# anonymousauthors001/SGS-GNN

Measured on AMD Instinct MI355X. Metric: sampled edges/sec + training steps/sec, Reddit hybrid 20% sparsity, higher is better.
Workload: dtype f32

## Files before the change

include/sgs_hip.h:

```cpp
#ifndef SGS_HIP_H_
#define SGS_HIP_H_

#include <stddef.h>
#include <stdint.h>

#ifdef __cplusplus
extern "C" {
#endif

#define SGS_ABI_VERSION 1

#define SGS_OK 0
#define SGS_EINVAL (-1)
#define SGS_EWORKSPACE (-2)
#define SGS_EHIP (-3)

typedef void* sgs_stream_t;

int sgs_abi_version(void);
const char* sgs_last_error(void);

int sgs_rng_set_epoch_buffer(const uint64_t* epoch_dev);
int sgs_exp_noise(uint64_t seed, uint64_t stream_id, int64_t E, float* noise, sgs_stream_t stream);
int sgs_dropout_keep(uint64_t seed, uint32_t site, int64_t rows, int64_t cols, float p, uint8_t* keep,
// ... 104 lines not shown
                          const int32_t* loop_eid, const int64_t* edge_index, const float* Hn, float* dw,
                          sgs_stream_t stream);

#define SGS_ACT_NONE 0
#define SGS_ACT_RELU 1
#define SGS_ACT_RELU_DROPOUT 2
int sgs_spmm_csr(const float* X, int64_t N, int64_t D, int64_t nnz, const int32_t* ptr, const int32_t* col, const float* val,
                 const float* diag, const float* bias, int act, float p_drop, uint64_t seed, uint32_t site, float* Y,
                 sgs_stream_t stream);

int sgs_sddmm_csr(const float* A, const float* B, int64_t N, int64_t D, int64_t nnz, const int32_t* ptr, const int32_t* col,
                  const int32_t* eid, float* g, float* gdiag, sgs_stream_t stream);

int sgs_spmm_csr_variant(int64_t N, int64_t D, int64_t nnz, int aligned16);
int sgs_sddmm_csr_variant(int64_t N, int64_t D, int64_t nnz, int aligned16);

int sgs_act_bwd(const float* dY, const float* Y, int64_t n, int act, float p_drop, float* dZ, sgs_stream_t stream);
size_t sgs_colsum_workspace_bytes(int64_t N, int64_t D);
int sgs_colsum(const float* A, int64_t N, int64_t D, float* out, void* ws, size_t ws_bytes, sgs_stream_t stream);
int sgs_act_bwd_colsum(const float* dY, const float* Y, int64_t N, int64_t D, int act, float p_drop, float* dZ, float* colsum, void* ws,
                       size_t ws_bytes, sgs_stream_t stream);

int sgs_colsum_variant(int64_t N, int64_t D, int fused_act);

int sgs_gcn_pair_ok(int64_t N, int64_t nnz, int64_t D);
int sgs_spmm_csr_next(const float* X, int64_t N, int64_t D, int64_t nnz, const int32_t* ptr, const int32_t* col, const float* val,
                      const float* diag, const float* bias, int act, float p_drop, uint64_t seed, uint32_t site, const float* Wn, int64_t Dn,
                      float* Y, float* Z, sgs_stream_t stream);
int sgs_spmm_csr_bwd_prev(const float* dZ, int64_t N, int64_t D, int64_t nnz, const int32_t* ptr, const int32_t* col, const float* val,
                          const float* diag, const float* W, int64_t Dp, const float* Yp, int act, float p_drop, float* dX, float* dZp,
// ... 370 lines not shown
```

sgs-gnn_amd/csrc/gcn.hip:

```cpp
#include "sgs_common.h"

namespace sgs {
size_t graph_sort_workspace_bytes(int64_t n, int64_t N);
size_t graph_src_sorted_workspace_bytes(int64_t n, int64_t N);
int graph_build_src_sorted(const int64_t* ei, int64_t n, int64_t N, int32_t* in_ptr, int32_t* in_src, int32_t* in_eid, int32_t* out_ptr,
                           int32_t* out_dst, int32_t* out_eid, int32_t* loop_eid, int32_t* unsorted_flag, void* ws, size_t ws_bytes,
                           hipStream_t stream);
int graph_build_by_sort(const int64_t* ei, int64_t n, int64_t N, int32_t* in_ptr, int32_t* in_src, int32_t* in_eid, int32_t* out_ptr,
                        int32_t* out_dst, int32_t* out_eid, int32_t* loop_eid, void* ws, size_t ws_bytes, hipStream_t stream);
}

namespace sgs {
namespace {

constexpr int kT = 256;
constexpr int kMaxLdsRow = 8192;

__global__ void __launch_bounds__(kT) count_degrees(const int64_t* __restrict__ ei, int64_t n_edges, int* __restrict__ cnt_in,
                                                   int* __restrict__ cnt_out, int* __restrict__ loop_eid) {
    const int64_t e = static_cast<int64_t>(blockIdx.x) * kT + threadIdx.x;
    if (e >= n_edges) return;
    const int s = static_cast<int>(ei[e]), d = static_cast<int>(ei[n_edges + e]);
    atomicAdd(&cnt_in[d], 1);
    atomicAdd(&cnt_out[s], 1);
// ... 591 lines not shown
                        ? y * drop_scale : 0.f;
            o[v] = y;
        }
        *reinterpret_cast<V*>(Y + i * D + c0) = *reinterpret_cast<V*>(o);
    }
}
template <int VEC, int LPR>
__global__ void __launch_bounds__(kT) spmm_csr(const float* __restrict__ X, int64_t N, int64_t D, const int* __restrict__ ptr,
                                              const int* __restrict__ col, const float* __restrict__ val,
                                              const float* __restrict__ diag, const float* __restrict__ bias, int act,
                                              float drop_scale, uint32_t drop_thresh, uint64_t seed, uint32_t site,
                                              const uint64_t* __restrict__ epoch, float* __restrict__ Y) {
    spmm_csr_body<VEC, LPR>(X, N, D, ptr, col, val, diag, bias, act, drop_scale, drop_thresh, seed, site, epoch, Y);
}

template <int VEC, int NW>
__device__ __forceinline__ void spmm_csr_rowblock_body(const float* __restrict__ X, int64_t N, int64_t D, const int* __restrict__ ptr,
                                                       const int* __restrict__ col, const float* __restrict__ val,
                                                       const float* __restrict__ diag, const float* __restrict__ bias, int act,
                                                       float drop_scale, uint32_t drop_thresh, uint64_t seed, uint32_t site,
                                                       const uint64_t* __restrict__ epoch, float* __restrict__ Y) {
    using V = typename VecT<VEC>::type;
    __shared__ float part[NW][64 * VEC];
    seed = fold_epoch(seed, epoch);
    const int lane = threadIdx.x & 63, wave = threadIdx.x >> 6;
    const int64_t i = blockIdx.x;
    const int b = ptr[i], e = ptr[i + 1];
    const float dg = diag ? diag[i] : 0.f;
    const uint32_t rkey = dropout_row_key(seed, site, static_cast<uint64_t>(i));
    for (int64_t cbase = 0; cbase < D; cbase += 64 * VEC) {
        const int64_t c0 = cbase + static_cast<int64_t>(lane) * VEC;
        const bool in = c0 < D;
        float acc[VEC];
#pragma unroll
        for (int v = 0; v < VEC; ++v) acc[v] = 0.f;
        if (in) {
            int k = b + wave;
            for (; k + 7 * NW < e; k += 8 * NW) {
                int j[8]; float w[8]; V x[8];
#pragma unroll
                for (int u = 0; u < 8; ++u) { j[u] = col[k + NW * u]; w[u] = val[k + NW * u]; }
#pragma unroll
                for (int u = 0; u < 8; ++u) x[u] = *reinterpret_cast<const V*>(X + static_cast<int64_t>(j[u]) * D + c0);
#pragma unroll
                for (int u = 0; u < 8; ++u) {
                    float xv[VEC];
                    *reinterpret_cast<V*>(xv) = x[u];
#pragma unroll
                    for (int v = 0; v < VEC; ++v) acc[v] = fmaf(w[u], xv[v], acc[v]);
                }
            }
// ... 11 lines not shown
        const int t = threadIdx.x;
        if (t < 64 * VEC && cbase + t < D) {
            const int64_t c = cbase + t;
            float y = 0.f;
#pragma unroll
            for (int g = 0; g < NW; g += 4) y += (part[g][t] + part[g + 1][t]) + (part[g + 2][t] + part[g + 3][t]);
            if (diag) y = fmaf(dg, X[i * D + c], y);
            if (bias) y += bias[c];
            if (act != SGS_ACT_NONE) y = fmaxf(y, 0.f);
            if (act == SGS_ACT_RELU_DROPOUT) y = dropout_keep_col(rkey, static_cast<uint32_t>(c), drop_thresh) ? y * drop_scale : 0.f;
            Y[i * D + c] = y;
        }
        __syncthreads();
    }
}
template <int VEC, int NW>
__global__ void __launch_bounds__(64 * NW) spmm_csr_rowblock(const float* __restrict__ X, int64_t N, int64_t D, const int* __restrict__ ptr,
                                                       const int* __restrict__ col, const float* __restrict__ val,
                                                       const float* __restrict__ diag, const float* __restrict__ bias, int act,
                                                       float drop_scale, uint32_t drop_thresh, uint64_t seed, uint32_t site,
                                                       const uint64_t* __restrict__ epoch, float* __restrict__ Y) {
    spmm_csr_rowblock_body<VEC, NW>(X, N, D, ptr, col, val, diag, bias, act, drop_scale, drop_thresh, seed, site, epoch, Y);
}

template <int VEC, int LPR>
__global__ void __launch_bounds__(kT) sddmm_csr(const float* __restrict__ A, const float* __restrict__ B, int64_t N, int64_t D,
                                               const int* __restrict__ ptr, const int* __restrict__ col,
                                               const int* __restrict__ eid, float* __restrict__ g, float* __restrict__ gdiag) {
    using V = typename VecT<VEC>::type;
    constexpr int RPB = kT / LPR;
    const int sub = threadIdx.x % LPR;
    const int64_t i = static_cast<int64_t>(blockIdx.x) * RPB + threadIdx.x / LPR;
    const bool live = i < N;
    const int b = live ? ptr[i] : 0, e = live ? ptr[i + 1] : 0;
    int trips = e - b + 1;
    for (int o = 32; o > 0; o >>= 1) trips = max(trips, __shfl_xor(trips, o, 64));
    for (int t = 0; t < trips; ++t) {
// ... 260 lines not shown
__global__ void __launch_bounds__(kT) multi_norm_weights(const float* __restrict__ w, int64_t q, int64_t N, const int* __restrict__ in_ptr,
                                                        const int* __restrict__ in_src, const int* __restrict__ in_eid, const float* __restrict__ dis,
                                                        const float* __restrict__ loopw, float* __restrict__ what_in, float* __restrict__ what_loop) {
    const int64_t d = blockIdx.y;
    norm_weights_body(N, w ? w + d * q : nullptr, N, q, in_ptr + d * (N + 1), in_src + d * q, in_eid + d * q, nullptr, nullptr, nullptr, dis + d * N,
                      loopw + d * N, what_in + d * q, nullptr, what_loop + d * N);
}
template <int VEC, int LPR>
__global__ void __launch_bounds__(kT) multi_spmm_csr(const float* __restrict__ X, int64_t xs, int64_t N, int64_t D, int64_t nnz,
                                                    const int* __restrict__ ptr, const int* __restrict__ col, const float* __restrict__ val,
                                                    const float* __restrict__ diag, const float* __restrict__ bias, int act, float* __restrict__ Y) {
    const int64_t d = blockIdx.y;
    spmm_csr_body<VEC, LPR>(X + d * xs, N, D, ptr + d * (N + 1), col + d * nnz, val + d * nnz, diag ? diag + d * N : nullptr, bias, act, 1.0f, 0u,
                            uint64_t(0), 0u, nullptr, Y + d * N * D);
}
template <int VEC, int NW>
__global__ void __launch_bounds__(64 * NW) multi_spmm_csr_rowblock(const float* __restrict__ X, int64_t xs, int64_t N, int64_t D, int64_t nnz,
                                                                 const int* __restrict__ ptr, const int* __restrict__ col,
                                                                 const float* __restrict__ val, const float* __restrict__ diag,
                                                                 const float* __restrict__ bias, int act, float* __restrict__ Y) {
    const int64_t d = blockIdx.y;
    spmm_csr_rowblock_body<VEC, NW>(X + d * xs, N, D, ptr + d * (N + 1), col + d * nnz, val + d * nnz, diag ? diag + d * N : nullptr, bias, act,
                                    1.0f, 0u, uint64_t(0), 0u, nullptr, Y + d * N * D);
}

enum { kPairCol = 0, kPairFwd = 1, kPairBwd = 2 };
constexpr int kPairMaxD = 512;
constexpr int kPairWlds = 12288;
constexpr int kPairWpre = kPairWlds / 1024;
template <class FY, class FW>
__device__ __forceinline__ float lib_gemm_dot(int K, FY y, FW w) {
    const int Kmain = K / 16 * 16;
    float z = 0.f;
    if (Kmain > 0) {
        float ya[8], wa[8];
#pragma unroll
        for (int u = 0; u < 8; ++u) { const int k = 2 * (u & 3) + (u >> 2); ya[u] = y(k); wa[u] = w(k); }
        for (int b = 0; b < Kmain; b += 8) {
            const int nb = b + 8 < Kmain ? b + 8 : b;
            float yn[8], wn[8];
#pragma unroll
            for (int u = 0; u < 8; ++u) { const int k = nb + 2 * (u & 3) + (u >> 2); yn[u] = y(k); wn[u] = w(k); }
#pragma unroll
            for (int u = 0; u < 8; ++u) z = fmaf(ya[u], wa[u], z);
#pragma unroll
            for (int u = 0; u < 8; ++u) { ya[u] = yn[u]; wa[u] = wn[u]; }
        }
    }
    for (int k = Kmain; k < K; ++k) z = fmaf(y(k), w(k), z);
    return z;
}
template <int VEC, int NW, int MODE, int GU = 8>
__device__ __forceinline__ void spmm_rowgroup_pair_body(const float* __restrict__ X, int64_t N, int64_t D, const int* __restrict__ ptr,
                                                        const int* __restrict__ col, const float* __restrict__ val,
                                                        const float* __restrict__ diag, const float* __restrict__ bias, int act,
                                                        float drop_scale, uint32_t drop_thresh, uint64_t seed, uint32_t site,
                                                        const uint64_t* __restrict__ epoch, float* __restrict__ Y,
                                                        const float* __restrict__ Wn, int64_t Dn, const float* __restrict__ Yp,
                                                        float* __restrict__ Zn, int ncs, float* __restrict__ colsum) {
    using V = typename VecT<VEC>::type;
    constexpr int RG = 16 / NW;
    __shared__ float part[RG][NW][64 * VEC];
    __shared__ __align__(16) float ys[RG * kPairMaxD];
    __shared__ float wl[MODE == kPairFwd ? kPairWlds : 1];
    if (MODE != kPairFwd && static_cast<int>(blockIdx.x) < ncs) {
        if (D % 4 == 0) colsum_small_v4_body<false>(X, nullptr, N, D, SGS_ACT_NONE, 1.f, nullptr, colsum, blockIdx.x);
        else            colsum_small_body<false>(X, nullptr, N, D, SGS_ACT_NONE, 1.f, nullptr, colsum, blockIdx.x);
// ... 17 lines not shown
    const bool wlds = MODE == kPairFwd && Dn * D <= kPairWlds;
    float wpre[MODE == kPairFwd ? kPairWpre : 1];
    if (MODE == kPairFwd && wlds) {
#pragma unroll
        for (int u = 0; u < kPairWpre; ++u) {
            const int64_t idx = threadIdx.x + 1024 * u;
            wpre[u] = idx < Dn * D ? Wn[idx] : 0.f;
        }
    }
    for (int64_t cbase = 0; cbase < D; cbase += 64 * VEC) {
        const int64_t c0 = cbase + static_cast<int64_t>(lane) * VEC;
        const bool in = c0 < D;
        float acc[VEC];
#pragma unroll
        for (int v = 0; v < VEC; ++v) acc[v] = 0.f;
        if (in) {
            int k = b + wave;
            for (; k + (GU - 1) * NW < e; k += GU * NW) {
                int j[GU]; float w[GU]; V x[GU];
#pragma unroll
                for (int u = 0; u < GU; ++u) { j[u] = col[k + NW * u]; w[u] = val[k + NW * u]; }
#pragma unroll
                for (int u = 0; u < GU; ++u) x[u] = *reinterpret_cast<const V*>(X + static_cast<int64_t>(j[u]) * D + c0);
#pragma unroll
                for (int u = 0; u < GU; ++u) {
                    float xv[VEC];
                    *reinterpret_cast<V*>(xv) = x[u];
#pragma unroll
                    for (int v = 0; v < VEC; ++v) acc[v] = fmaf(w[u], xv[v], acc[v]);
                }
            }
// ... 44 lines not shown
            Zn[ir * Dn + o] = wlds ? lib_gemm_dot(static_cast<int>(D), yk, [&](int k) { return wl[k * Dn + o]; })
                                   : lib_gemm_dot(static_cast<int>(D), yk, [&](int k) { return Wn[o * D + k]; });
        }
    } else if (MODE == kPairBwd) {
        for (int64_t idx = threadIdx.x; idx < RG * Dn; idx += 1024) {
            const int r = static_cast<int>(idx / Dn);
            const int64_t ep = idx - r * Dn, ir = row0 + r;
            if (ir >= N) break;
            const float* yr = ys + r * D;
            float a = lib_gemm_dot(static_cast<int>(D), [&](int c) { return yr[c]; }, [&](int c) { return Wn[c * Dn + ep]; });
            if (act != SGS_ACT_NONE) a = (Yp[ir * Dn + ep] > 0.f) ? (act == SGS_ACT_RELU_DROPOUT ? a * drop_scale : a) : 0.f;
            Zn[ir * Dn + ep] = a;
        }
    }
}
template <int VEC, int NW, int MODE>
__global__ void __launch_bounds__(1024) spmm_rowgroup_pair(const float* __restrict__ X, int64_t N, int64_t D, const int* __restrict__ ptr,
                                                           const int* __restrict__ col, const float* __restrict__ val,
                                                           const float* __restrict__ diag, const float* __restrict__ bias, int act,
                                                           float drop_scale, uint32_t drop_thresh, uint64_t seed, uint32_t site,
                                                           const uint64_t* __restrict__ epoch, float* __restrict__ Y,
                                                           const float* __restrict__ Wn, int64_t Dn, const float* __restrict__ Yp,
                                                           float* __restrict__ Zn, int ncs, float* __restrict__ colsum) {
    spmm_rowgroup_pair_body<VEC, NW, MODE>(X, N, D, ptr, col, val, diag, bias, act, drop_scale, drop_thresh, seed, site, epoch, Y, Wn, Dn, Yp, Zn,
                                           ncs, colsum);
}

struct SpmmDualJob {
    const float* X;
    const int* ptr;
    const int* col;
    const float* val;
    const float* diag;
    float* Y;
    float* Z;
    int64_t nnz;
    uint64_t seed;
};
struct SpmmDualArgs {
    SpmmDualJob job[2];
};
template <int VEC, int NW>
__global__ void __launch_bounds__(64 * NW) spmm_csr_rowblock_dual(SpmmDualArgs a, int64_t N, int64_t D, const float* __restrict__ bias, int act,
                                                                  float drop_scale, uint32_t drop_thresh, uint32_t site,
                                                                  const uint64_t* __restrict__ epoch) {
    const SpmmDualJob& j = a.job[blockIdx.y];
    spmm_csr_rowblock_body<VEC, NW>(j.X, N, D, j.ptr, j.col, j.val, j.diag, bias, act, drop_scale, drop_thresh, j.seed, site, epoch, j.Y);
}
#ifndef SGS_DUAL_PAIR_CAPPED
#define SGS_DUAL_PAIR_CAPPED 1
#endif
constexpr int kDualPairWaves = SGS_DUAL_PAIR_CAPPED ? 8 : 4;
constexpr int dual_pair_gu(int vec) { return SGS_DUAL_PAIR_CAPPED && vec == 4 ? 4 : 8; }
template <int VEC, int NW>
__global__ void __launch_bounds__(1024, kDualPairWaves) spmm_rowgroup_pair_dual(SpmmDualArgs a, int64_t N, int64_t D,
                                                                                const float* __restrict__ bias, int act, float drop_scale,
                                                                                uint32_t drop_thresh, uint32_t site,
                                                                                const uint64_t* __restrict__ epoch,
                                                                                const float* __restrict__ Wn, int64_t Dn) {
    const SpmmDualJob& j = a.job[blockIdx.y];
    spmm_rowgroup_pair_body<VEC, NW, kPairFwd, dual_pair_gu(VEC)>(j.X, N, D, j.ptr, j.col, j.val, j.diag, bias, act, drop_scale, drop_thresh, j.seed,
                                                            site, epoch, j.Y, Wn, Dn, nullptr, j.Z, 0, nullptr);
}

inline int pick_lpr(int64_t D, int vec) {
    const int64_t need = (D + vec - 1) / vec;
    int lpr = 1;
    while (lpr < need && lpr < 64) lpr <<= 1;
    return lpr;
}

}
}

using namespace sgs;

#define DISPATCH_VEC_LPR(KERNEL, vec, lpr, grid_rows, ...)                                                       \
// ... 12 lines not shown
            }                                                                                                     \
        } else {                                                                                                  \
            switch (lpr) {                                                                                        \
                case 1: hipLaunchKernelGGL((KERNEL<1, 1>), _g, _b, 0, stream, __VA_ARGS__); break;                \
                case 2: hipLaunchKernelGGL((KERNEL<1, 2>), _g, _b, 0, stream, __VA_ARGS__); break;                \
                case 4: hipLaunchKernelGGL((KERNEL<1, 4>), _g, _b, 0, stream, __VA_ARGS__); break;                \
                case 8: hipLaunchKernelGGL((KERNEL<1, 8>), _g, _b, 0, stream, __VA_ARGS__); break;                \
                case 16: hipLaunchKernelGGL((KERNEL<1, 16>), _g, _b, 0, stream, __VA_ARGS__); break;              \
                case 32: hipLaunchKernelGGL((KERNEL<1, 32>), _g, _b, 0, stream, __VA_ARGS__); break;              \
                default: hipLaunchKernelGGL((KERNEL<1, 64>), _g, _b, 0, stream, __VA_ARGS__); break;              \
            }                                                                                                     \
        }                                                                                                         \
    } while (0)

static inline bool aligned16(const void* p) { return (reinterpret_cast<uintptr_t>(p) & 15) == 0; }

extern "C" {

constexpr int64_t kSortEdges = int64_t(1) << 22;

size_t sgs_graph_build_workspace_bytes(int64_t n_edges, int64_t N) {
    if (n_edges < 0) n_edges = 0;
    if (N < 0) N = 0;
    if (n_edges >= kSortEdges) return graph_sort_workspace_bytes(n_edges, N);
    return 4 * carve_bytes(N + 1, 4) + 2 * carve_bytes(n_edges + 1, 4) + 512;
}

int sgs_graph_build(const int64_t* edge_index, int64_t n_edges, int64_t N, int32_t* in_ptr, int32_t* in_src,
                    int32_t* in_eid, int32_t* out_ptr, int32_t* out_dst, int32_t* out_eid, int32_t* loop_eid, void* ws,
                    size_t ws_bytes, sgs_stream_t stream_) {
// ... 271 lines not shown
    SGS_REQUIRE(N >= 0 && n_edges >= 0, SGS_EINVAL, "sgs_gcn_norm_bwd_edge: bad sizes");
    if (n_edges == 0) return SGS_OK;
    SGS_REQUIRE(gw_hat && gloop && dis && loop_eid && edge_index && Hn && dw, SGS_EINVAL, "sgs_gcn_norm_bwd_edge: null pointer");
    hipLaunchKernelGGL(norm_bwd_edge, dim3(cdiv(n_edges, kT)), dim3(kT), 0, stream, gw_hat, gloop, edge_index, n_edges, loop_eid, dis, Hn, dw);
    SGS_LAUNCH_OK();
    return SGS_OK;
}

int sgs_spmm_csr_variant(int64_t N, int64_t D, int64_t nnz, int al16) {
    const int vec = (D % 4 == 0 && al16) ? 4 : 1;
    if (N <= 65536 && nnz >= 16 * N)
        return 1000 + vec * 100 + (nnz >= 256 * N ? 16 : 4);
    return vec * 100 + pick_lpr(D, vec);
}

int sgs_sddmm_csr_variant(int64_t N, int64_t D, int64_t nnz, int al16) {
    const int vec = (D % 4 == 0 && al16) ? 4 : 1;
    if (nnz >= 16 * N)
        return 1000 + vec * 100 + (nnz >= 64 * N ? 16 : 4);
    return vec * 100 + pick_lpr(D, vec);
}

int sgs_spmm_csr(const float* X, int64_t N, int64_t D, int64_t nnz, const int32_t* ptr, const int32_t* col, const float* val,
                 const float* diag, const float* bias, int act, float p_drop, uint64_t seed, uint32_t site, float* Y,
                 sgs_stream_t stream_) {
    hipStream_t stream = static_cast<hipStream_t>(stream_);
    SGS_REQUIRE(N >= 0 && D >= 0, SGS_EINVAL, "sgs_spmm_csr: bad sizes");
    SGS_REQUIRE(act >= SGS_ACT_NONE && act <= SGS_ACT_RELU_DROPOUT && p_drop >= 0.f && p_drop < 1.f, SGS_EINVAL,
                "sgs_spmm_csr: bad activation / dropout");
    if (N == 0 || D == 0) return SGS_OK;
    SGS_REQUIRE(X && ptr && Y && X != Y, SGS_EINVAL, "sgs_spmm_csr: null or aliased pointer");
    const int var = sgs_spmm_csr_variant(N, D, nnz, aligned16(X) && aligned16(Y));
    const float scale = 1.0f / (1.0f - p_drop);
    const uint32_t th = dropout_thresh(p_drop);
    if (act == SGS_ACT_RELU_DROPOUT && p_drop == 0.f) act = SGS_ACT_RELU;
    const dim3 g_(static_cast<unsigned>(N));
    switch (var) {
        case 1416:
            hipLaunchKernelGGL((spmm_csr_rowblock<4, 16>), g_, dim3(1024), 0, stream, X, N, D, ptr, col, val, diag, bias, act, scale, th, seed,
                               site, epoch_ptr(), Y);
            break;
        case 1404:
            hipLaunchKernelGGL((spmm_csr_rowblock<4, 4>), g_, dim3(kT), 0, stream, X, N, D, ptr, col, val, diag, bias, act, scale, th, seed,
                               site, epoch_ptr(), Y);
            break;
        case 1116:
            hipLaunchKernelGGL((spmm_csr_rowblock<1, 16>), g_, dim3(1024), 0, stream, X, N, D, ptr, col, val, diag, bias, act, scale, th, seed,
                               site, epoch_ptr(), Y);
            break;
        case 1104:
            hipLaunchKernelGGL((spmm_csr_rowblock<1, 4>), g_, dim3(kT), 0, stream, X, N, D, ptr, col, val, diag, bias, act, scale, th, seed,
                               site, epoch_ptr(), Y);
            break;
        default: {
            const int vec = var / 100, lpr = var % 100;
            DISPATCH_VEC_LPR(spmm_csr, vec, lpr, N, X, N, D, ptr, col, val, diag, bias, act, scale, th, seed, site, epoch_ptr(), Y);
        }
    }
    SGS_LAUNCH_OK();
    return SGS_OK;
}

int sgs_sddmm_csr(const float* A, const float* B, int64_t N, int64_t D, int64_t nnz, const int32_t* ptr, const int32_t* col,
                  const int32_t* eid, float* g, float* gdiag, sgs_stream_t stream_) {
    hipStream_t stream = static_cast<hipStream_t>(stream_);
    SGS_REQUIRE(N >= 0 && D >= 0, SGS_EINVAL, "sgs_sddmm_csr: bad sizes");
// ... 88 lines not shown
        case 2:
            hipLaunchKernelGGL(colsum_small_v4<true>, dim3(cdiv(D, 16)), dim3(1024), 0, stream, dY, Y, N, D, act, 1.0f / (1.0f - p_drop), dZ, colsum);
            break;
        default:
            if (int rc = sgs_act_bwd(dY, Y, N * D, act, p_drop, dZ, stream_)) return rc;
            return sgs_colsum(dZ, N, D, colsum, ws, ws_bytes, stream_);
    }
    SGS_LAUNCH_OK();
    return SGS_OK;
}

int sgs_gcn_pair_ok(int64_t N, int64_t nnz, int64_t D) {
    return (N > 0 && N <= 65536 && nnz >= 16 * N && D > 0 && D <= kPairMaxD) ? 1 : 0;
}

#define PAIR_LAUNCH(MODE, grid, ...)                                                                                              \
    do {                                                                                                                          \
        if (vec == 4 && wide)  hipLaunchKernelGGL((spmm_rowgroup_pair<4, 16, MODE>), dim3(grid), dim3(1024), 0, stream, __VA_ARGS__); \
        else if (vec == 4)     hipLaunchKernelGGL((spmm_rowgroup_pair<4, 4, MODE>), dim3(grid), dim3(1024), 0, stream, __VA_ARGS__);  \
        else if (wide)         hipLaunchKernelGGL((spmm_rowgroup_pair<1, 16, MODE>), dim3(grid), dim3(1024), 0, stream, __VA_ARGS__); \
        else                   hipLaunchKernelGGL((spmm_rowgroup_pair<1, 4, MODE>), dim3(grid), dim3(1024), 0, stream, __VA_ARGS__);  \
    } while (0)

int sgs_spmm_csr_next(const float* X, int64_t N, int64_t D, int64_t nnz, const int32_t* ptr, const int32_t* col, const float* val,
                      const float* diag, const float* bias, int act, float p_drop, uint64_t seed, uint32_t site, const float* Wn, int64_t Dn,
                      float* Y, float* Z, sgs_stream_t stream_) {
    hipStream_t stream = static_cast<hipStream_t>(stream_);
    SGS_REQUIRE(sgs_gcn_pair_ok(N, nnz, D) && Dn > 0, SGS_EINVAL, "sgs_spmm_csr_next: not a row-block shape (see sgs_gcn_pair_ok)");
    SGS_REQUIRE(act >= SGS_ACT_NONE && act <= SGS_ACT_RELU_DROPOUT && p_drop >= 0.f && p_drop < 1.f, SGS_EINVAL,
                "sgs_spmm_csr_next: bad activation / dropout");
    SGS_REQUIRE(X && ptr && Y && Wn && Z && X != Y && Z != Y && Z != X, SGS_EINVAL, "sgs_spmm_csr_next: null or aliased pointer");
    const int vec = (D % 4 == 0 && aligned16(X) && aligned16(Y)) ? 4 : 1;
    const bool wide = nnz >= 256 * N;
    const float scale = 1.0f / (1.0f - p_drop);
    const uint32_t th = dropout_thresh(p_drop);
    if (act == SGS_ACT_RELU_DROPOUT && p_drop == 0.f) act = SGS_ACT_RELU;
    const int64_t grid = cdiv(N, wide ? 1 : 4);
    PAIR_LAUNCH(kPairFwd, grid, X, N, D, ptr, col, val, diag, bias, act, scale, th, seed, site, epoch_ptr(), Y, Wn, Dn,
                static_cast<const float*>(nullptr), Z, 0, static_cast<float*>(nullptr));
    SGS_LAUNCH_OK();
    return SGS_OK;
}

int sgs_spmm_csr_bwd_prev(const float* dZ, int64_t N, int64_t D, int64_t nnz, const int32_t* ptr, const int32_t* col, const float* val,
                          const float* diag, const float* W, int64_t Dp, const float* Yp, int act, float p_drop, float* dX, float* dZp,
                          float* colsum, sgs_stream_t stream_) {
    hipStream_t stream = static_cast<hipStream_t>(stream_);
    SGS_REQUIRE(sgs_gcn_pair_ok(N, nnz, D), SGS_EINVAL, "sgs_spmm_csr_bwd_prev: not a row-block shape (see sgs_gcn_pair_ok)");
    SGS_REQUIRE(act >= SGS_ACT_NONE && act <= SGS_ACT_RELU_DROPOUT && p_drop >= 0.f && p_drop < 1.f, SGS_EINVAL,
                "sgs_spmm_csr_bwd_prev: bad activation / dropout");
    SGS_REQUIRE(dZ && ptr && dX && dZ != dX, SGS_EINVAL, "sgs_spmm_csr_bwd_prev: null or aliased pointer");
    SGS_REQUIRE(!W || (Dp > 0 && dZp && (act == SGS_ACT_NONE || Yp) && dZp != dX && dZp != dZ), SGS_EINVAL,
                "sgs_spmm_csr_bwd_prev: W needs Dp > 0, dZp and (with an activation) Yp");
    const int vec = (D % 4 == 0 && aligned16(dZ) && aligned16(dX)) ? 4 : 1;
    const bool wide = nnz >= 256 * N;
    const int ncs = colsum ? static_cast<int>(cdiv(D, 16)) : 0;
    const int64_t grid = ncs + cdiv(N, wide ? 1 : 4);
    const float scale = 1.0f / (1.0f - p_drop);
    if (W)
        PAIR_LAUNCH(kPairBwd, grid, dZ, N, D, ptr, col, val, diag, static_cast<const float*>(nullptr), act, scale, 0u, uint64_t(0), 0u,
                    static_cast<const uint64_t*>(nullptr), dX, W, Dp, Yp, dZp, ncs, colsum);
    else
        PAIR_LAUNCH(kPairCol, grid, dZ, N, D, ptr, col, val, diag, static_cast<const float*>(nullptr), SGS_ACT_NONE, 1.f, 0u, uint64_t(0), 0u,
                    static_cast<const uint64_t*>(nullptr), dX, static_cast<const float*>(nullptr), int64_t(0), static_cast<const float*>(nullptr),
                    static_cast<float*>(nullptr), ncs, colsum);
    SGS_LAUNCH_OK();
    return SGS_OK;
}
#undef PAIR_LAUNCH

int sgs_gcn_dual_ok(int64_t N, int64_t nnz_a, int64_t nnz_b, int64_t D, int64_t Dn) {
    return (sgs_gcn_pair_ok(N, nnz_a, D) && sgs_gcn_pair_ok(N, nnz_b, D) && Dn > 0 && (nnz_a >= 256 * N) == (nnz_b >= 256 * N)) ? 1 : 0;
}

int sgs_spmm_csr_next_dual(const float* X, int64_t N, int64_t D, const float* bias, int act, float p_drop, uint32_t site, const float* Wn,
                           int64_t Dn, int64_t nnz_a, const int32_t* ptr_a, const int32_t* col_a, const float* val_a, const float* diag_a,
                           uint64_t seed_a, float* Y_a, float* Z_a, int64_t nnz_b, const int32_t* ptr_b, const int32_t* col_b,
                           const float* val_b, const float* diag_b, uint64_t seed_b, float* Y_b, float* Z_b, sgs_stream_t stream_) {
    hipStream_t stream = static_cast<hipStream_t>(stream_);
    SGS_REQUIRE(sgs_gcn_dual_ok(N, nnz_a, nnz_b, D, Dn), SGS_EINVAL, "sgs_spmm_csr_next_dual: not two row-block shapes of one variant (see sgs_gcn_dual_ok)");
    SGS_REQUIRE(act >= SGS_ACT_NONE && act <= SGS_ACT_RELU_DROPOUT && p_drop >= 0.f && p_drop < 1.f, SGS_EINVAL,
                "sgs_spmm_csr_next_dual: bad activation / dropout");
    SGS_REQUIRE(X && ptr_a && ptr_b && Y_a && Y_b && Wn && Z_a && Z_b && X != Y_a && X != Y_b && X != Z_a && X != Z_b && Y_a != Y_b &&
                    Z_a != Z_b && Y_a != Z_a && Y_a != Z_b && Y_b != Z_a && Y_b != Z_b,
                SGS_EINVAL, "sgs_spmm_csr_next_dual: null or aliased pointer");
    const int vec = (D % 4 == 0 && aligned16(X) && aligned16(Y_a)) ? 4 : 1;
    SGS_REQUIRE(vec == ((D % 4 == 0 && aligned16(X) && aligned16(Y_b)) ? 4 : 1), SGS_EINVAL,
                "sgs_spmm_csr_next_dual: the two jobs select different kernel variants (alignment)");
    const bool wide = nnz_a >= 256 * N;
    const float scale = 1.0f / (1.0f - p_drop);
    const uint32_t th = dropout_thresh(p_drop);
    if (act == SGS_ACT_RELU_DROPOUT && p_drop == 0.f) act = SGS_ACT_RELU;
    SpmmDualArgs a;
    a.job[0] = SpmmDualJob{X, ptr_a, col_a, val_a, diag_a, Y_a, Z_a, nnz_a, seed_a};
    a.job[1] = SpmmDualJob{X, ptr_b, col_b, val_b, diag_b, Y_b, Z_b, nnz_b, seed_b};
    const dim3 grid(static_cast<unsigned>(cdiv(N, wide ? 1 : 4)), 2);
    if (vec == 4 && wide)  hipLaunchKernelGGL((spmm_rowgroup_pair_dual<4, 16>), grid, dim3(1024), 0, stream, a, N, D, bias, act, scale, th, site, epoch_ptr(), Wn, Dn);
    else if (vec == 4)     hipLaunchKernelGGL((spmm_rowgroup_pair_dual<4, 4>), grid, dim3(1024), 0, stream, a, N, D, bias, act, scale, th, site, epoch_ptr(), Wn, Dn);
    else if (wide)         hipLaunchKernelGGL((spmm_rowgroup_pair_dual<1, 16>), grid, dim3(1024), 0, stream, a, N, D, bias, act, scale, th, site, epoch_ptr(), Wn, Dn);
    else                   hipLaunchKernelGGL((spmm_rowgroup_pair_dual<1, 4>), grid, dim3(1024), 0, stream, a, N, D, bias, act, scale, th, site, epoch_ptr(), Wn, Dn);
    SGS_LAUNCH_OK();
    return SGS_OK;
}

int sgs_spmm_csr_dual(const float* X_a, const float* X_b, int64_t N, int64_t D, const float* bias, int act, float p_drop, uint32_t site,
                      int64_t nnz_a, const int32_t* ptr_a, const int32_t* col_a, const float* val_a, const float* diag_a, uint64_t seed_a,
                      float* Y_a, int64_t nnz_b, const int32_t* ptr_b, const int32_t* col_b, const float* val_b, const float* diag_b,
                      uint64_t seed_b, float* Y_b, sgs_stream_t stream_) {
    hipStream_t stream = static_cast<hipStream_t>(stream_);
    SGS_REQUIRE(N > 0 && D > 0, SGS_EINVAL, "sgs_spmm_csr_dual: bad sizes");
    SGS_REQUIRE(act >= SGS_ACT_NONE && act <= SGS_ACT_RELU_DROPOUT && p_drop >= 0.f && p_drop < 1.f, SGS_EINVAL,
                "sgs_spmm_csr_dual: bad activation / dropout");
    SGS_REQUIRE(X_a && X_b && ptr_a && ptr_b && Y_a && Y_b && Y_a != Y_b && X_a != Y_a && X_a != Y_b && X_b != Y_a && X_b != Y_b, SGS_EINVAL,
                "sgs_spmm_csr_dual: null or aliased pointer");
    const int var = sgs_spmm_csr_variant(N, D, nnz_a, aligned16(X_a) && aligned16(Y_a));
    SGS_REQUIRE(var >= 1000 && var == sgs_spmm_csr_variant(N, D, nnz_b, aligned16(X_b) && aligned16(Y_b)), SGS_EINVAL,
                "sgs_spmm_csr_dual: not two row-block shapes of one variant (see sgs_spmm_csr_variant)");
    const float scale = 1.0f / (1.0f - p_drop);
    const uint32_t th = dropout_thresh(p_drop);
    if (act == SGS_ACT_RELU_DROPOUT && p_drop == 0.f) act = SGS_ACT_RELU;
    SpmmDualArgs a;
    a.job[0] = SpmmDualJob{X_a, ptr_a, col_a, val_a, diag_a, Y_a, nullptr, nnz_a, seed_a};
    a.job[1] = SpmmDualJob{X_b, ptr_b, col_b, val_b, diag_b, Y_b, nullptr, nnz_b, seed_b};
    const dim3 g_(static_cast<unsigned>(N), 2);
    switch (var) {
        case 1416: hipLaunchKernelGGL((spmm_csr_rowblock_dual<4, 16>), g_, dim3(1024), 0, stream, a, N, D, bias, act, scale, th, site, epoch_ptr()); break;
        case 1404: hipLaunchKernelGGL((spmm_csr_rowblock_dual<4, 4>), g_, dim3(kT), 0, stream, a, N, D, bias, act, scale, th, site, epoch_ptr()); break;
        case 1116: hipLaunchKernelGGL((spmm_csr_rowblock_dual<1, 16>), g_, dim3(1024), 0, stream, a, N, D, bias, act, scale, th, site, epoch_ptr()); break;
        default:   hipLaunchKernelGGL((spmm_csr_rowblock_dual<1, 4>), g_, dim3(kT), 0, stream, a, N, D, bias, act, scale, th, site, epoch_ptr()); break;
    }
    SGS_LAUNCH_OK();
    return SGS_OK;
}

}

extern "C" {

size_t sgs_graph_filter_multi_workspace_bytes(int64_t E_parent, int64_t N, int64_t D) {
    if (E_parent < 0) E_parent = 0;
    if (N < 0) N = 0;
    if (D < 1) D = 1;
    return 2 * carve_bytes(static_cast<size_t>(D * (N + 1)), 4) + carve_bytes(static_cast<size_t>(D * E_parent + 1), 4) + 256;
}
// ... 73 lines not shown
int sgs_spmm_csr_multi(const float* X, int64_t x_stride, int64_t N, int64_t Dc, int64_t nnz, int64_t D, const int32_t* ptr, const int32_t* col,
                       const float* val, const float* diag, const float* bias, int act, float* Y, sgs_stream_t stream_) {
    hipStream_t stream = static_cast<hipStream_t>(stream_);
    SGS_REQUIRE(N >= 0 && Dc >= 0 && nnz >= 0 && D >= 1 && D <= 65535 && x_stride >= 0, SGS_EINVAL, "sgs_spmm_csr_multi: bad sizes");
    SGS_REQUIRE(act == SGS_ACT_NONE || act == SGS_ACT_RELU, SGS_EINVAL, "sgs_spmm_csr_multi: act must be NONE or RELU (forward only)");
    if (N == 0 || Dc == 0) return SGS_OK;
    SGS_REQUIRE(X && ptr && Y && (nnz == 0 || (col && val)), SGS_EINVAL, "sgs_spmm_csr_multi: null pointer");
    SGS_REQUIRE(x_stride == 0 || x_stride >= N * Dc, SGS_EINVAL, "sgs_spmm_csr_multi: x_stride must be 0 (shared X) or >= N * Dc");
    SGS_REQUIRE(X + (D - 1) * x_stride + N * Dc <= Y || Y + D * N * Dc <= X, SGS_EINVAL, "sgs_spmm_csr_multi: X and Y overlap");
    const int vec = (Dc % 4 == 0 && x_stride % 4 == 0 && aligned16(X) && aligned16(Y)) ? 4 : 1;
    const int lpr = pick_lpr(Dc, vec);
    const unsigned Du = static_cast<unsigned>(D);
    if (N <= 65536 && nnz >= 16 * N) {
        const bool wide = nnz >= 256 * N;
        const dim3 g_(static_cast<unsigned>(N), Du);
        if (vec == 4 && wide)
            hipLaunchKernelGGL((multi_spmm_csr_rowblock<4, 16>), g_, dim3(1024), 0, stream, X, x_stride, N, Dc, nnz, ptr, col, val, diag, bias, act, Y);
        else if (vec == 4)
            hipLaunchKernelGGL((multi_spmm_csr_rowblock<4, 4>), g_, dim3(kT), 0, stream, X, x_stride, N, Dc, nnz, ptr, col, val, diag, bias, act, Y);
        else if (wide)
            hipLaunchKernelGGL((multi_spmm_csr_rowblock<1, 16>), g_, dim3(1024), 0, stream, X, x_stride, N, Dc, nnz, ptr, col, val, diag, bias, act, Y);
        else
            hipLaunchKernelGGL((multi_spmm_csr_rowblock<1, 4>), g_, dim3(kT), 0, stream, X, x_stride, N, Dc, nnz, ptr, col, val, diag, bias, act, Y);
    } else {
        DISPATCH_VEC_LPR_Y(multi_spmm_csr, vec, lpr, N, Du, X, x_stride, N, Dc, nnz, ptr, col, val, diag, bias, act, Y);
    }
    SGS_LAUNCH_OK();
    return SGS_OK;
}

}
```

Baseline: 103.5 million.

## Add wave-cooperative long-row gather path to CSR SpMM kernels

Adds a specialised gather path for CSR rows with at least 256 nonzeros. Each lane prefetches one column index and weight, which are then broadcast with readlane, and the X row gathers are double-buffered in groups. The path is enabled through template flags across the rowblock, pair and dual kernels, but only when N ≤ 4096 and a global switch is on. The aim is to hide index-load latency and raise memory-level parallelism on dense rows, at the cost of extra kernel instantiations and register pressure.

```diff
diff --git a/include/sgs_hip.h b/include/sgs_hip.h
--- a/include/sgs_hip.h
+++ b/include/sgs_hip.h
@@ -142,6 +142,10 @@
 
 int sgs_spmm_csr_variant(int64_t N, int64_t D, int64_t nnz, int aligned16);
 int sgs_sddmm_csr_variant(int64_t N, int64_t D, int64_t nnz, int aligned16);
+
+int sgs_spmm_long_rows_set(int on);
+int sgs_spmm_long_rows_threshold(void);
+int sgs_spmm_long_rows_active(int64_t N, int64_t D);
 
 int sgs_act_bwd(const float* dY, const float* Y, int64_t n, int act, float p_drop, float* dZ, sgs_stream_t stream);
 size_t sgs_colsum_workspace_bytes(int64_t N, int64_t D);
diff --git a/sgs-gnn_amd/csrc/gcn.hip b/sgs-gnn_amd/csrc/gcn.hip
--- a/sgs-gnn_amd/csrc/gcn.hip
+++ b/sgs-gnn_amd/csrc/gcn.hip
@@ -629,7 +629,70 @@
     spmm_csr_body<VEC, LPR>(X, N, D, ptr, col, val, diag, bias, act, drop_scale, drop_thresh, seed, site, epoch, Y);
 }
 
-template <int VEC, int NW>
+constexpr int kSpmmLongRow = 256;
+template <int VEC, int NW, int GU, bool PIPE>
+__device__ __forceinline__ void spmm_long_row_gather(const float* __restrict__ X, int64_t D, const int* __restrict__ col,
+                                                     const float* __restrict__ val, int b, int e, int wave, int lane, int64_t cl,
+                                                     float (&acc)[VEC]) {
+    using V = typename VecT<VEC>::type;
+    const int k0 = __builtin_amdgcn_readfirstlane(b) + __builtin_amdgcn_readfirstlane(wave);
+    const int cnt = (__builtin_amdgcn_readfirstlane(e) - k0 + NW - 1) / NW;
+    const uint32_t cb = static_cast<uint32_t>(cl) * 4u;
+    const uint32_t rowb = static_cast<uint32_t>(D) * 4u;
+    const char* __restrict__ Xb = reinterpret_cast<const char*>(X);
+    constexpr int NG = 64 / GU;
+    int jn = 0;
+    float wn = 0.f;
+    if (lane < cnt) { jn = col[k0 + NW * lane]; wn = val[k0 + NW * lane]; }
+    for (int m0 = 0; m0 < cnt; m0 += 64) {
+        const uint32_t ol = static_cast<uint32_t>(jn) * rowb;
+        const float wl = wn;
+        const int mn = m0 + 64 + lane;
+        if (mn < cnt) { jn = col[k0 + NW * mn]; wn = val[k0 + NW * mn]; }
+        const int nb = cnt - m0 < 64 ? cnt - m0 : 64;
+        const int ng = nb / GU;
+        const auto ld = [&](int m) {
+            const uint32_t off = static_cast<uint32_t>(__builtin_amdgcn_readlane(static_cast<int>(ol), m)) + cb;
+            return *reinterpret_cast<const V*>(Xb + off);
+        };
+        const auto fm = [&](const V& x, int m) {
+            const float w = __builtin_bit_cast(float, __builtin_amdgcn_readlane(__builtin_bit_cast(int, wl), m));
+            float xv[VEC];
+            *reinterpret_cast<V*>(xv) = x;
+#pragma unroll
+            for (int v = 0; v < VEC; ++v) acc[v] = fmaf(w, xv[v], acc[v]);
+        };
+        V x[PIPE ? 2 : 1][GU];
+        if (PIPE && ng > 0) {
+#pragma unroll
+            for (int u = 0; u < GU; ++u) x[0][u] = ld(u);
+        }
+#pragma unroll
+        for (int g = 0; g < NG; ++g) {
+            if (g < ng) {
+                constexpr int one = PIPE ? 1 : 0;
+                if (PIPE) {
+                    if (g + 1 < ng) {
+#pragma unroll
+                        for (int u = 0; u < GU; ++u) x[(g + 1) & one][u] = ld((g + 1) * GU + u);
+                    }
+                } else {
+#pragma unroll
+                    for (int u = 0; u < GU; ++u) x[0][u] = ld(g * GU + u);
+                }
+#pragma unroll
+                for (int u = 0; u < GU; ++u) fm(x[g & one][u], g * GU + u);
+            }
+        }
+        const int t0 = ng * GU, rem = nb - t0;
+#pragma unroll
+        for (int u = 0; u < GU - 1; ++u) if (u < rem) x[0][u] = ld(t0 + u);
+#pragma unroll
+        for (int u = 0; u < GU - 1; ++u) if (u < rem) fm(x[0][u], t0 + u);
+    }
+}
+
+template <int VEC, int NW, bool LONG>
 __device__ __forceinline__ void spmm_csr_rowblock_body(const float* __restrict__ X, int64_t N, int64_t D, const int* __restrict__ ptr,
                                                        const int* __restrict__ col, const float* __restrict__ val,
                                                        const float* __restrict__ diag, const float* __restrict__ bias, int act,
@@ -649,7 +712,9 @@
         float acc[VEC];
 #pragma unroll
         for (int v = 0; v < VEC; ++v) acc[v] = 0.f;
-        if (in) {
+        if (LONG && e - b >= kSpmmLongRow) {
+            spmm_long_row_gather<VEC, NW, 8, true>(X, D, col, val, b, e, wave, lane, in ? c0 : 0, acc);
+        } else if (in) {
             int k = b + wave;
             for (; k + 7 * NW < e; k += 8 * NW) {
                 int j[8]; float w[8]; V x[8];
@@ -691,13 +756,13 @@
         __syncthreads();
     }
 }
-template <int VEC, int NW>
+template <int VEC, int NW, bool LONG>
 __global__ void __launch_bounds__(64 * NW) spmm_csr_rowblock(const float* __restrict__ X, int64_t N, int64_t D, const int* __restrict__ ptr,
                                                        const int* __restrict__ col, const float* __restrict__ val,
                                                        const float* __restrict__ diag, const float* __restrict__ bias, int act,
                                                        float drop_scale, uint32_t drop_thresh, uint64_t seed, uint32_t site,
                                                        const uint64_t* __restrict__ epoch, float* __restrict__ Y) {
-    spmm_csr_rowblock_body<VEC, NW>(X, N, D, ptr, col, val, diag, bias, act, drop_scale, drop_thresh, seed, site, epoch, Y);
+    spmm_csr_rowblock_body<VEC, NW, LONG>(X, N, D, ptr, col, val, diag, bias, act, drop_scale, drop_thresh, seed, site, epoch, Y);
 }
 
 template <int VEC, int LPR>
@@ -988,13 +1053,13 @@
     spmm_csr_body<VEC, LPR>(X + d * xs, N, D, ptr + d * (N + 1), col + d * nnz, val + d * nnz, diag ? diag + d * N : nullptr, bias, act, 1.0f, 0u,
                             uint64_t(0), 0u, nullptr, Y + d * N * D);
 }
-template <int VEC, int NW>
+template <int VEC, int NW, bool LONG>
 __global__ void __launch_bounds__(64 * NW) multi_spmm_csr_rowblock(const float* __restrict__ X, int64_t xs, int64_t N, int64_t D, int64_t nnz,
                                                                  const int* __restrict__ ptr, const int* __restrict__ col,
                                                                  const float* __restrict__ val, const float* __restrict__ diag,
                                                                  const float* __restrict__ bias, int act, float* __restrict__ Y) {
     const int64_t d = blockIdx.y;
-    spmm_csr_rowblock_body<VEC, NW>(X + d * xs, N, D, ptr + d * (N + 1), col + d * nnz, val + d * nnz, diag ? diag + d * N : nullptr, bias, act,
+    spmm_csr_rowblock_body<VEC, NW, LONG>(X + d * xs, N, D, ptr + d * (N + 1), col + d * nnz, val + d * nnz, diag ? diag + d * N : nullptr, bias, act,
                                     1.0f, 0u, uint64_t(0), 0u, nullptr, Y + d * N * D);
 }
 
@@ -1024,7 +1089,7 @@
     for (int k = Kmain; k < K; ++k) z = fmaf(y(k), w(k), z);
     return z;
 }
-template <int VEC, int NW, int MODE, int GU = 8>
+template <int VEC, int NW, int MODE, bool LONG, int GU = 8, int LGU = GU, bool LPIPE = true>
 __device__ __forceinline__ void spmm_rowgroup_pair_body(const float* __restrict__ X, int64_t N, int64_t D, const int* __restrict__ ptr,
                                                         const int* __restrict__ col, const float* __restrict__ val,
                                                         const float* __restrict__ diag, const float* __restrict__ bias, int act,
@@ -1072,7 +1137,9 @@
         float acc[VEC];
 #pragma unroll
         for (int v = 0; v < VEC; ++v) acc[v] = 0.f;
-        if (in) {
+        if (LONG && e - b >= kSpmmLongRow) {
+            spmm_long_row_gather<VEC, NW, LGU, LPIPE>(X, D, col, val, b, e, wave, lane, in ? c0 : 0, acc);
+        } else if (in) {
             int k = b + wave;
             for (; k + (GU - 1) * NW < e; k += GU * NW) {
                 int j[GU]; float w[GU]; V x[GU];
@@ -1147,7 +1214,7 @@
         }
     }
 }
-template <int VEC, int NW, int MODE>
+template <int VEC, int NW, int MODE, bool LONG>
 __global__ void __launch_bounds__(1024) spmm_rowgroup_pair(const float* __restrict__ X, int64_t N, int64_t D, const int* __restrict__ ptr,
                                                            const int* __restrict__ col, const float* __restrict__ val,
                                                            const float* __restrict__ diag, const float* __restrict__ bias, int act,
@@ -1155,7 +1222,7 @@
                                                            const uint64_t* __restrict__ epoch, float* __restrict__ Y,
                                                            const float* __restrict__ Wn, int64_t Dn, const float* __restrict__ Yp,
                                                            float* __restrict__ Zn, int ncs, float* __restrict__ colsum) {
-    spmm_rowgroup_pair_body<VEC, NW, MODE>(X, N, D, ptr, col, val, diag, bias, act, drop_scale, drop_thresh, seed, site, epoch, Y, Wn, Dn, Yp, Zn,
+    spmm_rowgroup_pair_body<VEC, NW, MODE, LONG>(X, N, D, ptr, col, val, diag, bias, act, drop_scale, drop_thresh, seed, site, epoch, Y, Wn, Dn, Yp, Zn,
                                            ncs, colsum);
 }
 
@@ -1173,27 +1240,30 @@
 struct SpmmDualArgs {
     SpmmDualJob job[2];
 };
-template <int VEC, int NW>
+template <int VEC, int NW, bool LONG>
 __global__ void __launch_bounds__(64 * NW) spmm_csr_rowblock_dual(SpmmDualArgs a, int64_t N, int64_t D, const float* __restrict__ bias, int act,
                                                                   float drop_scale, uint32_t drop_thresh, uint32_t site,
                                                                   const uint64_t* __restrict__ epoch) {
     const SpmmDualJob& j = a.job[blockIdx.y];
-    spmm_csr_rowblock_body<VEC, NW>(j.X, N, D, j.ptr, j.col, j.val, j.diag, bias, act, drop_scale, drop_thresh, j.seed, site, epoch, j.Y);
+    spmm_csr_rowblock_body<VEC, NW, LONG>(j.X, N, D, j.ptr, j.col, j.val, j.diag, bias, act, drop_scale, drop_thresh, j.seed, site, epoch, j.Y);
 }
 #ifndef SGS_DUAL_PAIR_CAPPED
 #define SGS_DUAL_PAIR_CAPPED 1
 #endif
 constexpr int kDualPairWaves = SGS_DUAL_PAIR_CAPPED ? 8 : 4;
 constexpr int dual_pair_gu(int vec) { return SGS_DUAL_PAIR_CAPPED && vec == 4 ? 4 : 8; }
-template <int VEC, int NW>
+constexpr bool dual_pair_long(int vec) { return !(SGS_DUAL_PAIR_CAPPED && vec == 4); }
+constexpr int dual_pair_long_gu(int vec) { return SGS_DUAL_PAIR_CAPPED ? 4 : 8; }
+template <int VEC, int NW, bool LONG>
 __global__ void __launch_bounds__(1024, kDualPairWaves) spmm_rowgroup_pair_dual(SpmmDualArgs a, int64_t N, int64_t D,
                                                                                 const float* __restrict__ bias, int act, float drop_scale,
                                                                                 uint32_t drop_thresh, uint32_t site,
                                                                                 const uint64_t* __restrict__ epoch,
                                                                                 const float* __restrict__ Wn, int64_t Dn) {
     const SpmmDualJob& j = a.job[blockIdx.y];
-    spmm_rowgroup_pair_body<VEC, NW, kPairFwd, dual_pair_gu(VEC)>(j.X, N, D, j.ptr, j.col, j.val, j.diag, bias, act, drop_scale, drop_thresh, j.seed,
-                                                            site, epoch, j.Y, Wn, Dn, nullptr, j.Z, 0, nullptr);
+    spmm_rowgroup_pair_body<VEC, NW, kPairFwd, LONG && dual_pair_long(VEC), dual_pair_gu(VEC), dual_pair_long_gu(VEC)>(j.X, N, D, j.ptr, j.col, j.val, j.diag, bias, act, drop_scale,
+                                                                                  drop_thresh, j.seed, site, epoch, j.Y, Wn, Dn, nullptr, j.Z, 0,
+                                                                                  nullptr);
 }
 
 inline int pick_lpr(int64_t D, int vec) {
@@ -1236,6 +1306,17 @@
     } while (0)
 
 static inline bool aligned16(const void* p) { return (reinterpret_cast<uintptr_t>(p) & 15) == 0; }
+
+static int g_spmm_long_rows = 1;
+constexpr int64_t kSpmmLongMaxRows = 4096;
+static inline bool spmm_long_rows_on(int64_t N, int64_t D) {
+    return g_spmm_long_rows && N <= kSpmmLongMaxRows && D <= (int64_t(1) << 18);
+}
+#define LAUNCH_LR(KERNEL, V_, W_, grid, block, ...)                                                              \
+    do {                                                                                                          \
+        if (lr) hipLaunchKernelGGL((KERNEL<V_, W_, true>), grid, block, __VA_ARGS__);                             \
+        else    hipLaunchKernelGGL((KERNEL<V_, W_, false>), grid, block, __VA_ARGS__);                            \
+    } while (0)
 
 extern "C" {
 
@@ -1537,6 +1618,14 @@
     return vec * 100 + pick_lpr(D, vec);
 }
 
+int sgs_spmm_long_rows_set(int on) {
+    const int prev = g_spmm_long_rows;
+    g_spmm_long_rows = on ? 1 : 0;
+    return prev;
+}
+int sgs_spmm_long_rows_threshold(void) { return kSpmmLongRow; }
+int sgs_spmm_long_rows_active(int64_t N, int64_t D) { return spmm_long_rows_on(N, D) ? 1 : 0; }
+
 int sgs_sddmm_csr_variant(int64_t N, int64_t D, int64_t nnz, int al16) {
     const int vec = (D % 4 == 0 && al16) ? 4 : 1;
     if (nnz >= 16 * N)
@@ -1558,21 +1647,22 @@
     const uint32_t th = dropout_thresh(p_drop);
     if (act == SGS_ACT_RELU_DROPOUT && p_drop == 0.f) act = SGS_ACT_RELU;
     const dim3 g_(static_cast<unsigned>(N));
+    const bool lr = spmm_long_rows_on(N, D);
     switch (var) {
         case 1416:
-            hipLaunchKernelGGL((spmm_csr_rowblock<4, 16>), g_, dim3(1024), 0, stream, X, N, D, ptr, col, val, diag, bias, act, scale, th, seed,
+            LAUNCH_LR(spmm_csr_rowblock, 4, 16, g_, dim3(1024), 0, stream, X, N, D, ptr, col, val, diag, bias, act, scale, th, seed,
                                site, epoch_ptr(), Y);
             break;
         case 1404:
-            hipLaunchKernelGGL((spmm_csr_rowblock<4, 4>), g_, dim3(kT), 0, stream, X, N, D, ptr, col, val, diag, bias, act, scale, th, seed,
+            LAUNCH_LR(spmm_csr_rowblock, 4, 4, g_, dim3(kT), 0, stream, X, N, D, ptr, col, val, diag, bias, act, scale, th, seed,
                                site, epoch_ptr(), Y);
             break;
         case 1116:
-            hipLaunchKernelGGL((spmm_csr_rowblock<1, 16>), g_, dim3(1024), 0, stream, X, N, D, ptr, col, val, diag, bias, act, scale, th, seed,
+            LAUNCH_LR(spmm_csr_rowblock, 1, 16, g_, dim3(1024), 0, stream, X, N, D, ptr, col, val, diag, bias, act, scale, th, seed,
                                site, epoch_ptr(), Y);
             break;
         case 1104:
-            hipLaunchKernelGGL((spmm_csr_rowblock<1, 4>), g_, dim3(kT), 0, stream, X, N, D, ptr, col, val, diag, bias, act, scale, th, seed,
+            LAUNCH_LR(spmm_csr_rowblock, 1, 4, g_, dim3(kT), 0, stream, X, N, D, ptr, col, val, diag, bias, act, scale, th, seed,
                                site, epoch_ptr(), Y);
             break;
         default: {
@@ -1691,12 +1781,17 @@
     return (N > 0 && N <= 65536 && nnz >= 16 * N && D > 0 && D <= kPairMaxD) ? 1 : 0;
 }
 
+#define PAIR_LAUNCH1(V_, W_, MODE, grid, ...)                                                                                             \
+    do {                                                                                                                          \
+        if (lr) hipLaunchKernelGGL((spmm_rowgroup_pair<V_, W_, MODE, true>), dim3(grid), dim3(1024), 0, stream, __VA_ARGS__);      \
+        else    hipLaunchKernelGGL((spmm_rowgroup_pair<V_, W_, MODE, false>), dim3(grid), dim3(1024), 0, stream, __VA_ARGS__);     \
+    } while (0)
 #define PAIR_LAUNCH(MODE, grid, ...)                                                                                              \
     do {                                                                                                                          \
-        if (vec == 4 && wide)  hipLaunchKernelGGL((spmm_rowgroup_pair<4, 16, MODE>), dim3(grid), dim3(1024), 0, stream, __VA_ARGS__); \
-        else if (vec == 4)     hipLaunchKernelGGL((spmm_rowgroup_pair<4, 4, MODE>), dim3(grid), dim3(1024), 0, stream, __VA_ARGS__);  \
-        else if (wide)         hipLaunchKernelGGL((spmm_rowgroup_pair<1, 16, MODE>), dim3(grid), dim3(1024), 0, stream, __VA_ARGS__); \
-        else                   hipLaunchKernelGGL((spmm_rowgroup_pair<1, 4, MODE>), dim3(grid), dim3(1024), 0, stream, __VA_ARGS__);  \
+        if (vec == 4 && wide)  PAIR_LAUNCH1(4, 16, MODE, grid, __VA_ARGS__); \
+        else if (vec == 4)     PAIR_LAUNCH1(4, 4, MODE, grid, __VA_ARGS__);  \
+        else if (wide)         PAIR_LAUNCH1(1, 16, MODE, grid, __VA_ARGS__); \
+        else                   PAIR_LAUNCH1(1, 4, MODE, grid, __VA_ARGS__);  \
     } while (0)
 
 int sgs_spmm_csr_next(const float* X, int64_t N, int64_t D, int64_t nnz, const int32_t* ptr, const int32_t* col, const float* val,
@@ -1713,6 +1808,7 @@
     const uint32_t th = dropout_thresh(p_drop);
     if (act == SGS_ACT_RELU_DROPOUT && p_drop == 0.f) act = SGS_ACT_RELU;
     const int64_t grid = cdiv(N, wide ? 1 : 4);
+    const bool lr = spmm_long_rows_on(N, D);
     PAIR_LAUNCH(kPairFwd, grid, X, N, D, ptr, col, val, diag, bias, act, scale, th, seed, site, epoch_ptr(), Y, Wn, Dn,
                 static_cast<const float*>(nullptr), Z, 0, static_cast<float*>(nullptr));
     SGS_LAUNCH_OK();
@@ -1734,6 +1830,7 @@
     const int ncs = colsum ? static_cast<int>(cdiv(D, 16)) : 0;
     const int64_t grid = ncs + cdiv(N, wide ? 1 : 4);
     const float scale = 1.0f / (1.0f - p_drop);
+    const bool lr = spmm_long_rows_on(N, D);
     if (W)
         PAIR_LAUNCH(kPairBwd, grid, dZ, N, D, ptr, col, val, diag, static_cast<const float*>(nullptr), act, scale, 0u, uint64_t(0), 0u,
                     static_cast<const uint64_t*>(nullptr), dX, W, Dp, Yp, dZp, ncs, colsum);
@@ -1745,6 +1842,7 @@
     return SGS_OK;
 }
 #undef PAIR_LAUNCH
+#undef PAIR_LAUNCH1
 
 int sgs_gcn_dual_ok(int64_t N, int64_t nnz_a, int64_t nnz_b, int64_t D, int64_t Dn) {
     return (sgs_gcn_pair_ok(N, nnz_a, D) && sgs_gcn_pair_ok(N, nnz_b, D) && Dn > 0 && (nnz_a >= 256 * N) == (nnz_b >= 256 * N)) ? 1 : 0;
@@ -1772,10 +1870,11 @@
     a.job[0] = SpmmDualJob{X, ptr_a, col_a, val_a, diag_a, Y_a, Z_a, nnz_a, seed_a};
     a.job[1] = SpmmDualJob{X, ptr_b, col_b, val_b, diag_b, Y_b, Z_b, nnz_b, seed_b};
     const dim3 grid(static_cast<unsigned>(cdiv(N, wide ? 1 : 4)), 2);
-    if (vec == 4 && wide)  hipLaunchKernelGGL((spmm_rowgroup_pair_dual<4, 16>), grid, dim3(1024), 0, stream, a, N, D, bias, act, scale, th, site, epoch_ptr(), Wn, Dn);
-    else if (vec == 4)     hipLaunchKernelGGL((spmm_rowgroup_pair_dual<4, 4>), grid, dim3(1024), 0, stream, a, N, D, bias, act, scale, th, site, epoch_ptr(), Wn, Dn);
-    else if (wide)         hipLaunchKernelGGL((spmm_rowgroup_pair_dual<1, 16>), grid, dim3(1024), 0, stream, a, N, D, bias, act, scale, th, site, epoch_ptr(), Wn, Dn);
-    else                   hipLaunchKernelGGL((spmm_rowgroup_pair_dual<1, 4>), grid, dim3(1024), 0, stream, a, N, D, bias, act, scale, th, site, epoch_ptr(), Wn, Dn);
+    const bool lr = spmm_long_rows_on(N, D);
+    if (vec == 4 && wide)  LAUNCH_LR(spmm_rowgroup_pair_dual, 4, 16, grid, dim3(1024), 0, stream, a, N, D, bias, act, scale, th, site, epoch_ptr(), Wn, Dn);
+    else if (vec == 4)     LAUNCH_LR(spmm_rowgroup_pair_dual, 4, 4, grid, dim3(1024), 0, stream, a, N, D, bias, act, scale, th, site, epoch_ptr(), Wn, Dn);
+    else if (wide)         LAUNCH_LR(spmm_rowgroup_pair_dual, 1, 16, grid, dim3(1024), 0, stream, a, N, D, bias, act, scale, th, site, epoch_ptr(), Wn, Dn);
+    else                   LAUNCH_LR(spmm_rowgroup_pair_dual, 1, 4, grid, dim3(1024), 0, stream, a, N, D, bias, act, scale, th, site, epoch_ptr(), Wn, Dn);
     SGS_LAUNCH_OK();
     return SGS_OK;
 }
@@ -1800,11 +1899,12 @@
     a.job[0] = SpmmDualJob{X_a, ptr_a, col_a, val_a, diag_a, Y_a, nullptr, nnz_a, seed_a};
     a.job[1] = SpmmDualJob{X_b, ptr_b, col_b, val_b, diag_b, Y_b, nullptr, nnz_b, seed_b};
     const dim3 g_(static_cast<unsigned>(N), 2);
+    const bool lr = spmm_long_rows_on(N, D);
     switch (var) {
-        case 1416: hipLaunchKernelGGL((spmm_csr_rowblock_dual<4, 16>), g_, dim3(1024), 0, stream, a, N, D, bias, act, scale, th, site, epoch_ptr()); break;
-        case 1404: hipLaunchKernelGGL((spmm_csr_rowblock_dual<4, 4>), g_, dim3(kT), 0, stream, a, N, D, bias, act, scale, th, site, epoch_ptr()); break;
-        case 1116: hipLaunchKernelGGL((spmm_csr_rowblock_dual<1, 16>), g_, dim3(1024), 0, stream, a, N, D, bias, act, scale, th, site, epoch_ptr()); break;
-        default:   hipLaunchKernelGGL((spmm_csr_rowblock_dual<1, 4>), g_, dim3(kT), 0, stream, a, N, D, bias, act, scale, th, site, epoch_ptr()); break;
+        case 1416: LAUNCH_LR(spmm_csr_rowblock_dual, 4, 16, g_, dim3(1024), 0, stream, a, N, D, bias, act, scale, th, site, epoch_ptr()); break;
+        case 1404: LAUNCH_LR(spmm_csr_rowblock_dual, 4, 4, g_, dim3(kT), 0, stream, a, N, D, bias, act, scale, th, site, epoch_ptr()); break;
+        case 1116: LAUNCH_LR(spmm_csr_rowblock_dual, 1, 16, g_, dim3(1024), 0, stream, a, N, D, bias, act, scale, th, site, epoch_ptr()); break;
+        default:   LAUNCH_LR(spmm_csr_rowblock_dual, 1, 4, g_, dim3(kT), 0, stream, a, N, D, bias, act, scale, th, site, epoch_ptr()); break;
     }
     SGS_LAUNCH_OK();
     return SGS_OK;
@@ -1908,14 +2008,15 @@
     if (N <= 65536 && nnz >= 16 * N) {
         const bool wide = nnz >= 256 * N;
         const dim3 g_(static_cast<unsigned>(N), Du);
+        const bool lr = spmm_long_rows_on(N, Dc);
         if (vec == 4 && wide)
-            hipLaunchKernelGGL((multi_spmm_csr_rowblock<4, 16>), g_, dim3(1024), 0, stream, X, x_stride, N, Dc, nnz, ptr, col, val, diag, bias, act, Y);
+            LAUNCH_LR(multi_spmm_csr_rowblock, 4, 16, g_, dim3(1024), 0, stream, X, x_stride, N, Dc, nnz, ptr, col, val, diag, bias, act, Y);
         else if (vec == 4)
-            hipLaunchKernelGGL((multi_spmm_csr_rowblock<4, 4>), g_, dim3(kT), 0, stream, X, x_stride, N, Dc, nnz, ptr, col, val, diag, bias, act, Y);
+            LAUNCH_LR(multi_spmm_csr_rowblock, 4, 4, g_, dim3(kT), 0, stream, X, x_stride, N, Dc, nnz, ptr, col, val, diag, bias, act, Y);
         else if (wide)
-            hipLaunchKernelGGL((multi_spmm_csr_rowblock<1, 16>), g_, dim3(1024), 0, stream, X, x_stride, N, Dc, nnz, ptr, col, val, diag, bias, act, Y);
+            LAUNCH_LR(multi_spmm_csr_rowblock, 1, 16, g_, dim3(1024), 0, stream, X, x_stride, N, Dc, nnz, ptr, col, val, diag, bias, act, Y);
         else
-            hipLaunchKernelGGL((multi_spmm_csr_rowblock<1, 4>), g_, dim3(kT), 0, stream, X, x_stride, N, Dc, nnz, ptr, col, val, diag, bias, act, Y);
+            LAUNCH_LR(multi_spmm_csr_rowblock, 1, 4, g_, dim3(kT), 0, stream, X, x_stride, N, Dc, nnz, ptr, col, val, diag, bias, act, Y);
     } else {
         DISPATCH_VEC_LPR_Y(multi_spmm_csr, vec, lpr, N, Du, X, x_stride, N, Dc, nnz, ptr, col, val, diag, bias, act, Y);
     }
```

After: 107.5 million (median of 6 runs). +3.8%, better.
